# NVlabs/STEP

Measured on NVIDIA H100. Metric: clips/sec (T=32,224x224) STEP max_iter=3, higher is better.
Workload: dtype f16

## Files before the change

step_b200/build.py:

```python
import os
import subprocess
import sys
from concurrent.futures import ThreadPoolExecutor

HERE = os.path.dirname(os.path.abspath(__file__))
CSRC = os.path.join(HERE, "csrc")
OBJ = os.path.join(HERE, "_obj")
LIB = os.path.join(HERE, "libstep_b200.so")
NVCC = os.environ.get("NVCC", "/usr/local/cuda/bin/nvcc")
SOURCES = ["api.cu", "nms.cu", "roi.cu", "tubes.cu", "pool_layout.cu", "conv_simt.cu", "conv_umma.cu", "conv_halo.cu", "bottleneck_exit.cu", "train.cu", "optim.cu"]
FLAGS = ["-gencode", "arch=compute_90a,code=sm_90a", "-O3", "-std=c++17", "-lineinfo",
         "-Xcompiler", "-fPIC", "-Xptxas", "-v"]
NO_FMAD = {"nms.cu", "roi.cu", "tubes.cu", "train.cu", "optim.cu"}


def _deps(src):
    return [os.path.join(CSRC, src), os.path.join(CSRC, "common.cuh"), os.path.join(CSRC, "umma_ptx.cuh"),
            os.path.join(os.path.dirname(HERE), "include", "step_b200.h")]


def _stale(target, deps):
    if not os.path.exists(target):
        return True
    t = os.path.getmtime(target)
    return any(os.path.getmtime(d) > t for d in deps)


def _compile(src, verbose):
    obj = os.path.join(OBJ, src.replace(".cu", ".o"))
    if not _stale(obj, _deps(src)):
        return obj, ""
    cmd = [NVCC] + FLAGS + (["-fmad=false"] if src in NO_FMAD else []) + ["-c", os.path.join(CSRC, src), "-o", obj]
    r = subprocess.run(cmd, capture_output=True, text=True)
    if r.returncode != 0:
        raise RuntimeError("nvcc failed for %s:\n%s\n%s" % (src, r.stdout, r.stderr))
    return obj, r.stderr


def build(verbose=False):
    os.makedirs(OBJ, exist_ok=True)
    with ThreadPoolExecutor(max_workers=min(8, len(SOURCES))) as ex:
        res = list(ex.map(lambda s: _compile(s, verbose), SOURCES))
    objs = [o for o, _ in res]
    if verbose:
        for _, log in res:
            if log:
                print(log)
    if _stale(LIB, objs):
        cmd = [NVCC, "-shared"] + FLAGS[:2] + ["-o", LIB] + objs + ["-lcudart"]
        r = subprocess.run(cmd, capture_output=True, text=True)
        if r.returncode != 0:
            raise RuntimeError("link failed:\n%s\n%s" % (r.stdout, r.stderr))
    return LIB


if __name__ == "__main__":
    print(build(verbose="-v" in sys.argv))
```

step_b200/csrc/api.cu:

```cuda
#include <stdarg.h>
#include <string.h>

#include <atomic>

#include <stdlib.h>

#include "common.cuh"

namespace step {

static thread_local char g_err[512] = "";
static std::atomic<uint64_t> g_launches{0};

char* err_buf() { return g_err; }
void count_launch() { g_launches.fetch_add(1, std::memory_order_relaxed); }

int fail(int code, const char* fmt, ...) {
  va_list ap;
  va_start(ap, fmt);
  vsnprintf(g_err, sizeof(g_err), fmt, ap);
  va_end(ap);
  return code ? code : STEP_E_ARG;
}

int conv3d_simt_launch(const step_conv_params* p, step_stream_t stream);
int conv3d_umma_launch(const step_conv_params* p, step_stream_t stream);
int conv3d_halo_launch(const step_conv_params* p, step_stream_t stream);
bool conv3d_halo_supported(const step_conv_params* p);

}

using namespace step;

extern "C" int step_version(void) { return 100; }
extern "C" const char* step_last_error(void) { return g_err; }
extern "C" uint64_t step_launch_count(void) { return g_launches.load(std::memory_order_relaxed); }

extern "C" int step_conv3d_fwd(const step_conv_params* p, step_stream_t stream) {
  STEP_CHECK_ARG(p != nullptr, "conv3d: null params");
  STEP_CHECK_ARG(p->dtype == STEP_F32 || p->dtype == STEP_F16, "conv3d: bad dtype %d", p->dtype);
  STEP_CHECK_ARG(p->x && p->w && p->y, "conv3d: null tensor pointer");
  STEP_CHECK_ARG(p->N > 0 && p->T > 0 && p->H > 0 && p->W > 0 && p->Cin > 0 && p->Cout > 0, "conv3d: bad extent");
  STEP_CHECK_ARG(p->KT > 0 && p->KH > 0 && p->KW > 0 && p->ST > 0 && p->SH > 0 && p->SW > 0, "conv3d: bad filter/stride");
  STEP_CHECK_ARG(p->OT > 0 && p->OH > 0 && p->OW > 0, "conv3d: bad output extent");
  STEP_CHECK_ARG(p->n_splits >= 0 && p->n_splits <= 2, "conv3d: bad n_splits");
  STEP_CHECK_ARG(p->n_splits > 0 || p->out_ld >= p->out_coff + p->Cout, "conv3d: output slice [%d,%d) exceeds out_ld %d",
                 p->out_coff, p->out_coff + p->Cout, p->out_ld);
  STEP_CHECK_ARG(p->n_splits == 0 || (p->dtype == STEP_F16 && p->a_mode != 9), "conv3d: fused outputs are f16 tensor-core only");
  STEP_CHECK_ARG((p->OT - 1) * p->ST - p->PT < p->T && (p->OH - 1) * p->SH - p->PH < p->H && (p->OW - 1) * p->SW - p->PW < p->W,
                 "conv3d: output extent inconsistent with input/stride/pad");
  if (p->dtype == STEP_F32 || p->a_mode == 9) return conv3d_simt_launch(p, stream);
  if (p->a_mode == 4) {
    STEP_CHECK_ARG(p->ST == 1 && p->SH == 1 && p->SW == 1 && conv3d_halo_supported(p), "conv3d: a_mode 4 (halo) does not fit this problem");
    return conv3d_halo_launch(p, stream);
  }
  if (p->a_mode == 5) {
    static const bool halo_on = !(getenv("STEP_B200_HALO") && getenv("STEP_B200_HALO")[0] == '0');
    const int taps = p->KT * p->KH * p->KW;
    const int small = p->OH < p->OW ? p->OH : p->OW;
    if (halo_on && taps > 1 && p->ST == 1 && p->SH == 1 && p->SW == 1 && conv3d_halo_supported(p) &&
        p->Cin <= 32 && small >= 14)
      return conv3d_halo_launch(p, stream);
    step_conv_params q = *p;
    q.a_mode = taps == 1 ? 0 : 3;
    return conv3d_umma_launch(&q, stream);
  }
  return conv3d_umma_launch(p, stream);
}
```

step_b200/csrc/umma_ptx.cuh:

```cuda
#pragma once
#include <cuda.h>
#include <cuda_fp16.h>
#include <stdint.h>

namespace step {

__device__ __forceinline__ uint32_t smem_u32(const void* p) { return (uint32_t)__cvta_generic_to_shared(p); }

__device__ __forceinline__ void mbar_init(uint64_t* bar, uint32_t count) {
  asm volatile("mbarrier.init.shared::cta.b64 [%0], %1;" ::"r"(smem_u32(bar)), "r"(count));
}
__device__ __forceinline__ void mbar_expect_tx(uint64_t* bar, uint32_t bytes) {
  asm volatile("mbarrier.arrive.expect_tx.shared::cta.b64 _, [%0], %1;" ::"r"(smem_u32(bar)), "r"(bytes) : "memory");
}
__device__ __forceinline__ void mbar_arrive(uint64_t* bar) {
  asm volatile("mbarrier.arrive.shared::cta.b64 _, [%0];" ::"r"(smem_u32(bar)) : "memory");
}
__device__ __forceinline__ void mbar_wait(uint64_t* bar, uint32_t parity) {
  asm volatile(
      "{\n\t.reg .pred p;\n\t"
      "WAIT_LOOP:\n\t"
      "mbarrier.try_wait.parity.shared::cta.b64 p, [%0], %1;\n\t"
      "@p bra.uni WAIT_DONE;\n\t"
      "bra.uni WAIT_LOOP;\n\t"
      "WAIT_DONE:\n\t}" ::"r"(smem_u32(bar)), "r"(parity) : "memory");
}
__device__ __forceinline__ void fence_barrier_init() { asm volatile("fence.mbarrier_init.release.cluster;" ::: "memory"); }
__device__ __forceinline__ void fence_proxy_async() { asm volatile("fence.proxy.async.shared::cta;" ::: "memory"); }
__device__ __forceinline__ void named_sync(int id, int n) { asm volatile("bar.sync %0, %1;" ::"r"(id), "r"(n) : "memory"); }

__device__ __forceinline__ void tma_load_2d(const CUtensorMap* map, uint64_t* bar, void* dst, int c0, int c1) {
  asm volatile("cp.async.bulk.tensor.2d.shared::cluster.global.mbarrier::complete_tx::bytes [%0], [%1, {%3, %4}], [%2];"
               ::"r"(smem_u32(dst)), "l"(map), "r"(smem_u32(bar)), "r"(c0), "r"(c1) : "memory");
}
__device__ __forceinline__ void tma_load_3d(const CUtensorMap* map, uint64_t* bar, void* dst, int c0, int c1, int c2) {
  asm volatile("cp.async.bulk.tensor.3d.shared::cluster.global.mbarrier::complete_tx::bytes [%0], [%1, {%3, %4, %5}], [%2];"
               ::"r"(smem_u32(dst)), "l"(map), "r"(smem_u32(bar)), "r"(c0), "r"(c1), "r"(c2) : "memory");
}
__device__ __forceinline__ void tma_load_5d(const CUtensorMap* map, uint64_t* bar, void* dst, int c0, int c1, int c2,
                                            int c3, int c4) {
  asm volatile("cp.async.bulk.tensor.5d.shared::cluster.global.mbarrier::complete_tx::bytes [%0], [%1, {%3, %4, %5, %6, %7}], [%2];"
               ::"r"(smem_u32(dst)), "l"(map), "r"(smem_u32(bar)), "r"(c0), "r"(c1), "r"(c2), "r"(c3), "r"(c4) : "memory");
}
__device__ __forceinline__ void tma_load_im2col_5d(const CUtensorMap* map, uint64_t* bar, void* dst, int c, int w, int h,
                                                   int d, int n, uint16_t ow, uint16_t oh, uint16_t od) {
  asm volatile("cp.async.bulk.tensor.5d.shared::cluster.global.im2col.mbarrier::complete_tx::bytes [%0], [%1, {%3, %4, %5, %6, %7}], [%2], {%8, %9, %10};"
               ::"r"(smem_u32(dst)), "l"(map), "r"(smem_u32(bar)), "r"(c), "r"(w), "r"(h), "r"(d), "r"(n), "h"(ow), "h"(oh), "h"(od) : "memory");
}
__device__ __forceinline__ void tma_store_2d(const CUtensorMap* map, const void* src, int c0, int c1) {
  asm volatile("cp.async.bulk.tensor.2d.global.shared::cta.bulk_group [%0, {%2, %3}], [%1];"
               ::"l"(map), "r"(smem_u32(src)), "r"(c0), "r"(c1) : "memory");
}
__device__ __forceinline__ void bulk_commit() { asm volatile("cp.async.bulk.commit_group;" ::: "memory"); }
template <int N>
__device__ __forceinline__ void bulk_wait_read() { asm volatile("cp.async.bulk.wait_group.read %0;" ::"n"(N) : "memory"); }

template <int BK>
__device__ __forceinline__ uint64_t desc_hi_kmajor() {
  constexpr uint64_t sw = BK == 64 ? 1 : (BK == 32 ? 2 : 3);
  return (1ULL << 16) | ((uint64_t)((8 * BK * 2) >> 4) << 32) | (sw << 62);
}
__device__ __forceinline__ uint64_t desc_lo(const void* p) { return (uint64_t)((smem_u32(p) & 0x3FFFF) >> 4); }

__device__ __forceinline__ void wg_fence() { asm volatile("wgmma.fence.sync.aligned;" ::: "memory"); }
__device__ __forceinline__ void wg_commit() { asm volatile("wgmma.commit_group.sync.aligned;" ::: "memory"); }
template <int N>
__device__ __forceinline__ void wg_wait() { asm volatile("wgmma.wait_group.sync.aligned %0;" ::"n"(N) : "memory"); }

template <int N>
__device__ __forceinline__ void wgmma_f16(float* d, uint64_t da, uint64_t db, uint32_t accumulate);

#define STEP_D4(i) "+f"(d[4 * (i)]), "+f"(d[4 * (i) + 1]), "+f"(d[4 * (i) + 2]), "+f"(d[4 * (i) + 3])
#define STEP_WGMMA_F16(N, IA, IB, IC, REGS, ...)                                                                        \
  template <>                                                                                                          \
  __device__ __forceinline__ void wgmma_f16<N>(float* d, uint64_t da, uint64_t db, uint32_t accumulate) {              \
    asm volatile("{\n\t.reg .pred p;\n\tsetp.ne.b32 p, %" #IC ", 0;\n\t"                                              \
                 "wgmma.mma_async.sync.aligned.m64n" #N "k16.f32.f16.f16 {" REGS "}, %" #IA ", %" #IB ", p, 1, 1, 0, 0;\n\t}" \
                 : __VA_ARGS__ : "l"(da), "l"(db), "r"(accumulate));                                                    \
  }
STEP_WGMMA_F16(32, 16, 17, 18,
               "%0, %1, %2, %3, %4, %5, %6, %7, %8, %9, %10, %11, %12, %13, %14, %15",
               STEP_D4(0), STEP_D4(1), STEP_D4(2), STEP_D4(3))
STEP_WGMMA_F16(64, 32, 33, 34,
               "%0, %1, %2, %3, %4, %5, %6, %7, %8, %9, %10, %11, %12, %13, %14, %15, %16, %17, %18, %19, %20, %21, %22, "
               "%23, %24, %25, %26, %27, %28, %29, %30, %31",
               STEP_D4(0), STEP_D4(1), STEP_D4(2), STEP_D4(3), STEP_D4(4), STEP_D4(5), STEP_D4(6), STEP_D4(7))
STEP_WGMMA_F16(128, 64, 65, 66,
               "%0, %1, %2, %3, %4, %5, %6, %7, %8, %9, %10, %11, %12, %13, %14, %15, %16, %17, %18, %19, %20, %21, %22, "
               "%23, %24, %25, %26, %27, %28, %29, %30, %31, %32, %33, %34, %35, %36, %37, %38, %39, %40, %41, %42, %43, "
               "%44, %45, %46, %47, %48, %49, %50, %51, %52, %53, %54, %55, %56, %57, %58, %59, %60, %61, %62, %63",
               STEP_D4(0), STEP_D4(1), STEP_D4(2), STEP_D4(3), STEP_D4(4), STEP_D4(5), STEP_D4(6), STEP_D4(7),
               STEP_D4(8), STEP_D4(9), STEP_D4(10), STEP_D4(11), STEP_D4(12), STEP_D4(13), STEP_D4(14), STEP_D4(15))
STEP_WGMMA_F16(144, 72, 73, 74,
               "%0, %1, %2, %3, %4, %5, %6, %7, %8, %9, %10, %11, %12, %13, %14, %15, %16, %17, %18, %19, %20, %21, %22, "
               "%23, %24, %25, %26, %27, %28, %29, %30, %31, %32, %33, %34, %35, %36, %37, %38, %39, %40, %41, %42, %43, "
               "%44, %45, %46, %47, %48, %49, %50, %51, %52, %53, %54, %55, %56, %57, %58, %59, %60, %61, %62, %63, %64, "
               "%65, %66, %67, %68, %69, %70, %71",
               STEP_D4(0), STEP_D4(1), STEP_D4(2), STEP_D4(3), STEP_D4(4), STEP_D4(5), STEP_D4(6), STEP_D4(7),
               STEP_D4(8), STEP_D4(9), STEP_D4(10), STEP_D4(11), STEP_D4(12), STEP_D4(13), STEP_D4(14), STEP_D4(15),
               STEP_D4(16), STEP_D4(17))
STEP_WGMMA_F16(152, 76, 77, 78,
               "%0, %1, %2, %3, %4, %5, %6, %7, %8, %9, %10, %11, %12, %13, %14, %15, %16, %17, %18, %19, %20, %21, %22, "
               "%23, %24, %25, %26, %27, %28, %29, %30, %31, %32, %33, %34, %35, %36, %37, %38, %39, %40, %41, %42, %43, "
               "%44, %45, %46, %47, %48, %49, %50, %51, %52, %53, %54, %55, %56, %57, %58, %59, %60, %61, %62, %63, %64, "
               "%65, %66, %67, %68, %69, %70, %71, %72, %73, %74, %75",
               STEP_D4(0), STEP_D4(1), STEP_D4(2), STEP_D4(3), STEP_D4(4), STEP_D4(5), STEP_D4(6), STEP_D4(7),
               STEP_D4(8), STEP_D4(9), STEP_D4(10), STEP_D4(11), STEP_D4(12), STEP_D4(13), STEP_D4(14), STEP_D4(15),
               STEP_D4(16), STEP_D4(17), STEP_D4(18))
STEP_WGMMA_F16(160, 80, 81, 82,
               "%0, %1, %2, %3, %4, %5, %6, %7, %8, %9, %10, %11, %12, %13, %14, %15, %16, %17, %18, %19, %20, %21, %22, "
               "%23, %24, %25, %26, %27, %28, %29, %30, %31, %32, %33, %34, %35, %36, %37, %38, %39, %40, %41, %42, %43, "
               "%44, %45, %46, %47, %48, %49, %50, %51, %52, %53, %54, %55, %56, %57, %58, %59, %60, %61, %62, %63, %64, "
               "%65, %66, %67, %68, %69, %70, %71, %72, %73, %74, %75, %76, %77, %78, %79",
               STEP_D4(0), STEP_D4(1), STEP_D4(2), STEP_D4(3), STEP_D4(4), STEP_D4(5), STEP_D4(6), STEP_D4(7),
               STEP_D4(8), STEP_D4(9), STEP_D4(10), STEP_D4(11), STEP_D4(12), STEP_D4(13), STEP_D4(14), STEP_D4(15),
               STEP_D4(16), STEP_D4(17), STEP_D4(18), STEP_D4(19))
STEP_WGMMA_F16(176, 88, 89, 90,
               "%0, %1, %2, %3, %4, %5, %6, %7, %8, %9, %10, %11, %12, %13, %14, %15, %16, %17, %18, %19, %20, %21, %22, "
               "%23, %24, %25, %26, %27, %28, %29, %30, %31, %32, %33, %34, %35, %36, %37, %38, %39, %40, %41, %42, %43, "
               "%44, %45, %46, %47, %48, %49, %50, %51, %52, %53, %54, %55, %56, %57, %58, %59, %60, %61, %62, %63, %64, "
               "%65, %66, %67, %68, %69, %70, %71, %72, %73, %74, %75, %76, %77, %78, %79, %80, %81, %82, %83, %84, %85, "
               "%86, %87",
               STEP_D4(0), STEP_D4(1), STEP_D4(2), STEP_D4(3), STEP_D4(4), STEP_D4(5), STEP_D4(6), STEP_D4(7),
               STEP_D4(8), STEP_D4(9), STEP_D4(10), STEP_D4(11), STEP_D4(12), STEP_D4(13), STEP_D4(14), STEP_D4(15),
               STEP_D4(16), STEP_D4(17), STEP_D4(18), STEP_D4(19), STEP_D4(20), STEP_D4(21))
STEP_WGMMA_F16(192, 96, 97, 98,
               "%0, %1, %2, %3, %4, %5, %6, %7, %8, %9, %10, %11, %12, %13, %14, %15, %16, %17, %18, %19, %20, %21, %22, "
               "%23, %24, %25, %26, %27, %28, %29, %30, %31, %32, %33, %34, %35, %36, %37, %38, %39, %40, %41, %42, %43, "
               "%44, %45, %46, %47, %48, %49, %50, %51, %52, %53, %54, %55, %56, %57, %58, %59, %60, %61, %62, %63, %64, "
               "%65, %66, %67, %68, %69, %70, %71, %72, %73, %74, %75, %76, %77, %78, %79, %80, %81, %82, %83, %84, %85, "
               "%86, %87, %88, %89, %90, %91, %92, %93, %94, %95",
               STEP_D4(0), STEP_D4(1), STEP_D4(2), STEP_D4(3), STEP_D4(4), STEP_D4(5), STEP_D4(6), STEP_D4(7),
               STEP_D4(8), STEP_D4(9), STEP_D4(10), STEP_D4(11), STEP_D4(12), STEP_D4(13), STEP_D4(14), STEP_D4(15),
               STEP_D4(16), STEP_D4(17), STEP_D4(18), STEP_D4(19), STEP_D4(20), STEP_D4(21), STEP_D4(22), STEP_D4(23))
STEP_WGMMA_F16(208, 104, 105, 106,
               "%0, %1, %2, %3, %4, %5, %6, %7, %8, %9, %10, %11, %12, %13, %14, %15, %16, %17, %18, %19, %20, %21, %22, "
               "%23, %24, %25, %26, %27, %28, %29, %30, %31, %32, %33, %34, %35, %36, %37, %38, %39, %40, %41, %42, %43, "
               "%44, %45, %46, %47, %48, %49, %50, %51, %52, %53, %54, %55, %56, %57, %58, %59, %60, %61, %62, %63, %64, "
               "%65, %66, %67, %68, %69, %70, %71, %72, %73, %74, %75, %76, %77, %78, %79, %80, %81, %82, %83, %84, %85, "
               "%86, %87, %88, %89, %90, %91, %92, %93, %94, %95, %96, %97, %98, %99, %100, %101, %102, %103",
               STEP_D4(0), STEP_D4(1), STEP_D4(2), STEP_D4(3), STEP_D4(4), STEP_D4(5), STEP_D4(6), STEP_D4(7),
               STEP_D4(8), STEP_D4(9), STEP_D4(10), STEP_D4(11), STEP_D4(12), STEP_D4(13), STEP_D4(14), STEP_D4(15),
               STEP_D4(16), STEP_D4(17), STEP_D4(18), STEP_D4(19), STEP_D4(20), STEP_D4(21), STEP_D4(22), STEP_D4(23),
               STEP_D4(24), STEP_D4(25))
STEP_WGMMA_F16(224, 112, 113, 114,
               "%0, %1, %2, %3, %4, %5, %6, %7, %8, %9, %10, %11, %12, %13, %14, %15, %16, %17, %18, %19, %20, %21, %22, "
               "%23, %24, %25, %26, %27, %28, %29, %30, %31, %32, %33, %34, %35, %36, %37, %38, %39, %40, %41, %42, %43, "
               "%44, %45, %46, %47, %48, %49, %50, %51, %52, %53, %54, %55, %56, %57, %58, %59, %60, %61, %62, %63, %64, "
               "%65, %66, %67, %68, %69, %70, %71, %72, %73, %74, %75, %76, %77, %78, %79, %80, %81, %82, %83, %84, %85, "
               "%86, %87, %88, %89, %90, %91, %92, %93, %94, %95, %96, %97, %98, %99, %100, %101, %102, %103, %104, "
               "%105, %106, %107, %108, %109, %110, %111",
               STEP_D4(0), STEP_D4(1), STEP_D4(2), STEP_D4(3), STEP_D4(4), STEP_D4(5), STEP_D4(6), STEP_D4(7),
               STEP_D4(8), STEP_D4(9), STEP_D4(10), STEP_D4(11), STEP_D4(12), STEP_D4(13), STEP_D4(14), STEP_D4(15),
               STEP_D4(16), STEP_D4(17), STEP_D4(18), STEP_D4(19), STEP_D4(20), STEP_D4(21), STEP_D4(22), STEP_D4(23),
               STEP_D4(24), STEP_D4(25), STEP_D4(26), STEP_D4(27))
STEP_WGMMA_F16(256, 128, 129, 130,
               "%0, %1, %2, %3, %4, %5, %6, %7, %8, %9, %10, %11, %12, %13, %14, %15, %16, %17, %18, %19, %20, %21, %22, "
               "%23, %24, %25, %26, %27, %28, %29, %30, %31, %32, %33, %34, %35, %36, %37, %38, %39, %40, %41, %42, %43, "
               "%44, %45, %46, %47, %48, %49, %50, %51, %52, %53, %54, %55, %56, %57, %58, %59, %60, %61, %62, %63, %64, "
               "%65, %66, %67, %68, %69, %70, %71, %72, %73, %74, %75, %76, %77, %78, %79, %80, %81, %82, %83, %84, %85, "
               "%86, %87, %88, %89, %90, %91, %92, %93, %94, %95, %96, %97, %98, %99, %100, %101, %102, %103, %104, "
               "%105, %106, %107, %108, %109, %110, %111, %112, %113, %114, %115, %116, %117, %118, %119, %120, %121, "
               "%122, %123, %124, %125, %126, %127",
               STEP_D4(0), STEP_D4(1), STEP_D4(2), STEP_D4(3), STEP_D4(4), STEP_D4(5), STEP_D4(6), STEP_D4(7),
               STEP_D4(8), STEP_D4(9), STEP_D4(10), STEP_D4(11), STEP_D4(12), STEP_D4(13), STEP_D4(14), STEP_D4(15),
               STEP_D4(16), STEP_D4(17), STEP_D4(18), STEP_D4(19), STEP_D4(20), STEP_D4(21), STEP_D4(22), STEP_D4(23),
               STEP_D4(24), STEP_D4(25), STEP_D4(26), STEP_D4(27), STEP_D4(28), STEP_D4(29), STEP_D4(30), STEP_D4(31))
#undef STEP_WGMMA_F16

template <int N>
__device__ __forceinline__ void wgmma_f16_ra(float* d, const uint32_t* a, uint64_t db, uint32_t accumulate);
template <>
__device__ __forceinline__ void wgmma_f16_ra<256>(float* d, const uint32_t* a, uint64_t db, uint32_t accumulate) {
  asm volatile("{\n\t.reg .pred p;\n\tsetp.ne.b32 p, %133, 0;\n\t"
               "wgmma.mma_async.sync.aligned.m64n256k16.f32.f16.f16 {"
               "%0, %1, %2, %3, %4, %5, %6, %7, %8, %9, %10, %11, %12, %13, %14, %15, %16, %17, %18, %19, %20, %21, %22, "
               "%23, %24, %25, %26, %27, %28, %29, %30, %31, %32, %33, %34, %35, %36, %37, %38, %39, %40, %41, %42, %43, "
               "%44, %45, %46, %47, %48, %49, %50, %51, %52, %53, %54, %55, %56, %57, %58, %59, %60, %61, %62, %63, %64, "
               "%65, %66, %67, %68, %69, %70, %71, %72, %73, %74, %75, %76, %77, %78, %79, %80, %81, %82, %83, %84, %85, "
               "%86, %87, %88, %89, %90, %91, %92, %93, %94, %95, %96, %97, %98, %99, %100, %101, %102, %103, %104, "
               "%105, %106, %107, %108, %109, %110, %111, %112, %113, %114, %115, %116, %117, %118, %119, %120, %121, "
               "%122, %123, %124, %125, %126, %127}, {%128, %129, %130, %131}, %132, p, 1, 1, 0;\n\t}"
               : STEP_D4(0), STEP_D4(1), STEP_D4(2), STEP_D4(3), STEP_D4(4), STEP_D4(5), STEP_D4(6), STEP_D4(7),
                 STEP_D4(8), STEP_D4(9), STEP_D4(10), STEP_D4(11), STEP_D4(12), STEP_D4(13), STEP_D4(14), STEP_D4(15),
                 STEP_D4(16), STEP_D4(17), STEP_D4(18), STEP_D4(19), STEP_D4(20), STEP_D4(21), STEP_D4(22), STEP_D4(23),
                 STEP_D4(24), STEP_D4(25), STEP_D4(26), STEP_D4(27), STEP_D4(28), STEP_D4(29), STEP_D4(30), STEP_D4(31)
               : "r"(a[0]), "r"(a[1]), "r"(a[2]), "r"(a[3]), "l"(db), "r"(accumulate));
}
#undef STEP_D4

__device__ __forceinline__ void wgmma_64x64(float* d, uint64_t da, uint64_t db, uint32_t accumulate) {
  wgmma_f16<64>(d, da, db, accumulate);
}

template <int R>
__device__ __forceinline__ void setmaxnreg_dec() { asm volatile("setmaxnreg.dec.sync.aligned.u32 %0;" ::"n"(R)); }
template <int R>
__device__ __forceinline__ void setmaxnreg_inc() { asm volatile("setmaxnreg.inc.sync.aligned.u32 %0;" ::"n"(R)); }

__device__ __forceinline__ void pdl_wait() { asm volatile("griddepcontrol.wait;" ::: "memory"); }
__device__ __forceinline__ void pdl_launch_dependents() { asm volatile("griddepcontrol.launch_dependents;" ::: "memory"); }

__device__ __forceinline__ bool elect_one() {
  uint32_t pred;
  asm volatile(
      "{\n\t.reg .pred p;\n\t"
      "elect.sync _|p, 0xffffffff;\n\t"
      "selp.u32 %0, 1, 0, p;\n\t}"
      : "=r"(pred));
  return pred != 0;
}


}
```

step_b200/i3d.py:

```python
import torch

from . import _lib as L
from . import engine as E
from .engine import Act


def get_padding_shape(filter_shape, stride):
    pads = [E.same_pad(k, s) for k, s in zip(filter_shape, stride)]
    return pads[1] + pads[2] + pads[0]


class Unit3Dpy(torch.nn.Module):

    def __init__(self, in_channels, out_channels, kernel_size=(1, 1, 1), stride=(1, 1, 1), activation='relu',
                 padding='SAME', use_bias=False, use_bn=True):
        super(Unit3Dpy, self).__init__()
        if padding not in ('SAME', 'VALID'):
            raise ValueError('padding should be in [VALID|SAME] but got {}'.format(padding))
        self.padding = padding
        self.activation = activation
        self.use_bn = use_bn
        self.kernel_size = tuple(kernel_size)
        self.stride = tuple(stride)
        self.conv3d = torch.nn.Conv3d(in_channels, out_channels, kernel_size, stride=stride, bias=use_bias)
        if use_bn:
            self.batch3d = torch.nn.BatchNorm3d(out_channels)
        self._cache = {}

    def packed(self, code, s2d=False):
        bn = self.batch3d if self.use_bn else None
        tens = [self.conv3d.weight, self.conv3d.bias] + ([bn.weight, bn.bias, bn.running_mean, bn.running_var] if bn else [])
        key = (code, s2d) + E.params_key(*tens)
        hit = self._cache.get("k")
        if hit != key:
            w = E.pack_stem_s2d(self.conv3d.weight) if s2d else E.pack_conv_weight(self.conv3d.weight, code)
            scale, shift = E.fold_bn(bn, self.conv3d.bias, self.conv3d.out_channels, w.device)
            self._cache = {"k": key, "v": (w, scale, shift)}
        return self._cache["v"]

    def out_channels(self):
        return self.conv3d.out_channels

    def forward(self, x, out=None, residual=None):
        if not isinstance(x, Act):
            raise RuntimeError("step_b200.Unit3Dpy runs on engine.Act handles; use BaseNet / TwoBranchNet")
        relu = self.activation is not None
        if self.padding == 'VALID':
            pad_lo = (0, 0, 0)
            dims = tuple((d - k) // s + 1 for d, k, s in zip((x.T, x.H, x.W), self.kernel_size, self.stride))
        else:
            pad_lo, dims = None, None
        w, scale, shift = self.packed(x.code)
        if out is None:
            od = dims or E.same_out_dims((x.T, x.H, x.W), self.kernel_size, self.stride)
            out = Act.empty(x.N, od[0], od[1], od[2], self.conv3d.out_channels, x.code, x.device)
        return E.conv(x, w, scale, shift, out, self.kernel_size, self.stride, pad_lo, relu, residual, out_dims=dims, tag=self)

    def forward_s2d(self, x_s2d):
        w, scale, shift = self.packed(L.F16, s2d=True)
        out = Act.empty(x_s2d.N, x_s2d.T, x_s2d.H, x_s2d.W, self.conv3d.out_channels, L.F16, x_s2d.device)
        return E.conv(x_s2d, w, scale, shift, out, (4, 4, 4), (1, 1, 1), (1, 1, 1), self.activation is not None,
                      a_mode=L.A_HALO if E.STEM_HALO else None, out_dims=(x_s2d.T, x_s2d.H, x_s2d.W),
                      zero_cin_last_kt=4 * self.conv3d.in_channels, tag=("s2d", self))


class MaxPool3dTFPadding(torch.nn.Module):

    def __init__(self, kernel_size, stride=None, padding='SAME'):
        super(MaxPool3dTFPadding, self).__init__()
        self.kernel_size = tuple(kernel_size)
        self.stride = tuple(stride if stride is not None else kernel_size)
        if padding == 'SAME':
            self.padding_shape = get_padding_shape(self.kernel_size, self.stride)

    def forward(self, x, out=None):
        return E.maxpool(x, self.kernel_size, self.stride, out)


class Mixed(torch.nn.Module):

    def __init__(self, in_channels, out_channels):
        super(Mixed, self).__init__()
        o = out_channels
        self.branch_0 = Unit3Dpy(in_channels, o[0], kernel_size=(1, 1, 1))
        self.branch_1 = torch.nn.Sequential(Unit3Dpy(in_channels, o[1], kernel_size=(1, 1, 1)),
                                            Unit3Dpy(o[1], o[2], kernel_size=(3, 3, 3)))
        self.branch_2 = torch.nn.Sequential(Unit3Dpy(in_channels, o[3], kernel_size=(1, 1, 1)),
                                            Unit3Dpy(o[3], o[4], kernel_size=(3, 3, 3)))
        self.branch_3 = torch.nn.Sequential(MaxPool3dTFPadding(kernel_size=(3, 3, 3), stride=(1, 1, 1), padding='SAME'),
                                            Unit3Dpy(in_channels, o[5], kernel_size=(1, 1, 1)))
        self.out_plan = (o[0], o[2], o[4], o[5])

    def out_channels(self):
        return sum(self.out_plan)

    def forward(self, x, out=None):
        c0, c1, c2, c3 = self.out_plan
        if out is None:
            out = Act.empty(x.N, x.T, x.H, x.W, c0 + c1 + c2 + c3, x.code, x.device)
        if x.code == L.F16 and E.FUSE_1X1:
            return self._forward_fused(x, out)
        E.run_parallel(
            x.device,
            lambda: self.branch_1[1](self.branch_1[0](x), out=out.slice(c0, c1)),
            [lambda: self.branch_0(x, out=out.slice(0, c0)),
             lambda: self.branch_2[1](self.branch_2[0](x), out=out.slice(c0 + c1, c2)),
             lambda: self.branch_3[1](self.branch_3[0](x), out=out.slice(c0 + c1 + c2, c3))])
        return out


    def _fused_weights(self):
        units = (self.branch_0, self.branch_1[0], self.branch_2[0])
        parts = [u.packed(L.F16) for u in units]
        key = tuple(id(p[0]) for p in parts)
        c = self.__dict__.get("_fused")
        if c is None or c[0] != key:
            w = torch.cat([p[0] for p in parts], 0).contiguous()
            scale = torch.cat([p[1] for p in parts]).contiguous()
            shift = torch.cat([p[2] for p in parts]).contiguous()
            self.__dict__["_fused"] = (key, (w, scale, shift))
            c = self.__dict__["_fused"]
        return c[1]

    def _forward_fused(self, x, out):
        c0, c1, c2, c3 = self.out_plan
        w, scale, shift = self._fused_weights()
        m1 = self.branch_1[0].conv3d.out_channels
        m2 = self.branch_2[0].conv3d.out_channels
        t1 = Act.empty(x.N, x.T, x.H, x.W, m1, x.code, x.device)
        t2 = Act.empty(x.N, x.T, x.H, x.W, m2, x.code, x.device)

        def trunk():
            E.conv(x, w, scale, shift, out.slice(0, c0), (1, 1, 1), extra_outs=[t1, t2],
                   tag=[self.branch_0, self.branch_1[0], self.branch_2[0]])

        def tail():
            E.run_parallel(x.device,
                           lambda: self.branch_1[1](t1, out=out.slice(c0, c1)),
                           [lambda: self.branch_2[1](t2, out=out.slice(c0 + c1, c2))])
        E.run_parallel(x.device, lambda: (trunk(), tail()),
                       [lambda: self.branch_3[1](self.branch_3[0](x), out=out.slice(c0 + c1 + c2, c3))],
                       first_side=2)
        return out


class I3D_head(torch.nn.Module):

    def __init__(self):
        super(I3D_head, self).__init__()
        self.maxPool3d = MaxPool3dTFPadding(kernel_size=(1, 3, 3), stride=(1, 2, 2), padding='SAME')
        self.mixed_5b = Mixed(832, [256, 160, 320, 32, 128, 128])
        self.mixed_5c = Mixed(832, [384, 192, 384, 48, 128, 128])


def build_trunk_stages():
    return [
        Unit3Dpy(out_channels=64, in_channels=3, kernel_size=(7, 7, 7), stride=(2, 2, 2), padding='SAME'),
        MaxPool3dTFPadding(kernel_size=(1, 3, 3), stride=(1, 2, 2), padding='SAME'),
        Unit3Dpy(out_channels=64, in_channels=64, kernel_size=(1, 1, 1), padding='SAME'),
        Unit3Dpy(out_channels=192, in_channels=64, kernel_size=(3, 3, 3), padding='SAME'),
        MaxPool3dTFPadding(kernel_size=(1, 3, 3), stride=(1, 2, 2), padding='SAME'),
        Mixed(192, [64, 96, 128, 16, 32, 32]),
        Mixed(256, [128, 128, 192, 32, 96, 64]),
        MaxPool3dTFPadding(kernel_size=(3, 3, 3), stride=(2, 2, 2), padding='SAME'),
        Mixed(480, [192, 96, 208, 16, 48, 64]),
        Mixed(512, [160, 112, 224, 24, 64, 64]),
        Mixed(512, [128, 128, 256, 24, 64, 64]),
        Mixed(512, [112, 144, 288, 32, 64, 64]),
        Mixed(528, [256, 160, 320, 32, 128, 128]),
    ]
```

Before: 1089.

## Add dedicated warp-specialized WGMMA kernel for space-to-depth stem convolution

Adds a specialized stem conv kernel for the 7x7x7 stem after space-to-depth (Cin=24, 4x4x4 taps, 64 outputs). A TMA producer warp loads the input halo patch and streams the weights through a 6-stage mbarrier ring. Two consumer warpgroups run WGMMA directly on the shifted patch descriptors and write the epilogue through stmatrix staging. The Python side slices the s2d input to the real 24 channels, so the zero-padded last-kt channels are skipped. The halo path now dispatches to this kernel when the shape matches, adding a highly shape-specific code path.

Measured after the change: 1132, median of 6. +3.9%, better.

```diff
diff --git a/step_b200/build.py b/step_b200/build.py
--- a/step_b200/build.py
+++ b/step_b200/build.py
@@ -8,7 +8,7 @@
 OBJ = os.path.join(HERE, "_obj")
 LIB = os.path.join(HERE, "libstep_b200.so")
 NVCC = os.environ.get("NVCC", "/usr/local/cuda/bin/nvcc")
-SOURCES = ["api.cu", "nms.cu", "roi.cu", "tubes.cu", "pool_layout.cu", "conv_simt.cu", "conv_umma.cu", "conv_halo.cu", "bottleneck_exit.cu", "train.cu", "optim.cu"]
+SOURCES = ["api.cu", "nms.cu", "roi.cu", "tubes.cu", "pool_layout.cu", "conv_simt.cu", "conv_umma.cu", "conv_halo.cu", "conv_stem.cu", "bottleneck_exit.cu", "train.cu", "optim.cu"]
 FLAGS = ["-gencode", "arch=compute_90a,code=sm_90a", "-O3", "-std=c++17", "-lineinfo",
          "-Xcompiler", "-fPIC", "-Xptxas", "-v"]
 NO_FMAD = {"nms.cu", "roi.cu", "tubes.cu", "train.cu", "optim.cu"}
diff --git a/step_b200/csrc/api.cu b/step_b200/csrc/api.cu
--- a/step_b200/csrc/api.cu
+++ b/step_b200/csrc/api.cu
@@ -27,6 +27,8 @@
 int conv3d_umma_launch(const step_conv_params* p, step_stream_t stream);
 int conv3d_halo_launch(const step_conv_params* p, step_stream_t stream);
 bool conv3d_halo_supported(const step_conv_params* p);
+int conv3d_stem_launch(const step_conv_params* p, step_stream_t stream);
+bool conv3d_stem_supported(const step_conv_params* p);
 
 }
 
@@ -51,6 +53,7 @@
                  "conv3d: output extent inconsistent with input/stride/pad");
   if (p->dtype == STEP_F32 || p->a_mode == 9) return conv3d_simt_launch(p, stream);
   if (p->a_mode == 4) {
+    if (conv3d_stem_supported(p)) return conv3d_stem_launch(p, stream);
     STEP_CHECK_ARG(p->ST == 1 && p->SH == 1 && p->SW == 1 && conv3d_halo_supported(p), "conv3d: a_mode 4 (halo) does not fit this problem");
     return conv3d_halo_launch(p, stream);
   }
diff --git a/step_b200/csrc/conv_stem.cu b/step_b200/csrc/conv_stem.cu
--- /dev/null
+++ b/step_b200/csrc/conv_stem.cu
@@ -0,0 +1,230 @@
+#include <cuda.h>
+#include <stdlib.h>
+#include <string.h>
+
+#include "common.cuh"
+#include "umma_ptx.cuh"
+
+namespace step {
+
+constexpr int kStemThreads = 384;
+constexpr int kStemTT = 4, kStemTH = 16, kStemTW = 8;
+constexpr int kStemGroups = 3;
+constexpr int kStemHpT = kStemTT + 3, kStemHpH = kStemTH + 3, kStemHpW = kStemTW + 3;
+constexpr int kStemPlanePix = kStemHpH * kStemHpW;
+constexpr int kStemChunk = (kStemHpT * kStemPlanePix * 16 + 127) / 128 * 128;
+constexpr int kStemBlock = 64 * 16;
+constexpr int kStemStageBytes = kStemGroups * 8 * kStemBlock;
+constexpr int kStemStages = 6;
+constexpr int kStemSteps = 8;
+constexpr int kStemBook = 1024;
+constexpr int kStemPitch = 144;
+constexpr int kStemSmem = kStemBook + 1024 + kStemStages * kStemStageBytes + kStemGroups * kStemChunk;
+static_assert(kStemSmem <= 227 * 1024, "stem kernel exceeds shared memory");
+static_assert(kStemTT * kStemTH * kStemTW * kStemPitch <= kStemStages * kStemStageBytes, "staging tile exceeds the ring");
+constexpr uint64_t kStemAHi = ((uint64_t)((4 * kStemBlock) >> 4) << 16) | ((uint64_t)(128 >> 4) << 32);
+constexpr uint64_t kStemBHi = ((uint64_t)((kStemHpW * 16) >> 4) << 16) | ((uint64_t)((kStemHpW * 16) >> 4) << 32);
+
+struct StemGeom {
+  int OT, OH, OW, tiles_w, tiles_h, tiles_t;
+  int out_ld, out_coff, relu;
+};
+
+template <int NG>
+__device__ __forceinline__ void stem_mma_stage(float (&acc)[2][64], uint64_t a_lo, uint64_t b_lo) {
+#pragma unroll
+  for (int kw = 0; kw < 4; ++kw)
+#pragma unroll
+    for (int gi = 0; gi < NG; ++gi)
+#pragma unroll
+      for (int j = 0; j < 2; ++j)
+        wgmma_f16<128>(acc[j], kStemAHi | (a_lo + (uint64_t)((gi * 8 + kw) * (kStemBlock >> 4))),
+                       kStemBHi | (b_lo + (uint64_t)(gi * (kStemChunk >> 4) + j * kStemPlanePix + kw)), 1u);
+}
+
+template <int NG>
+__device__ __forceinline__ void stem_stage(float (&acc)[2][64], int st, int wg, bool leader, uint8_t* ring, uint8_t* patch,
+                                           uint64_t* full_bar, uint64_t* empty_bar) {
+  const int s = st % kStemStages;
+  mbar_wait(&full_bar[s], (uint32_t)(st / kStemStages) & 1u);
+  const int kt = st >> 1, kh0 = (st & 1) * 2;
+  const uint64_t a_lo = desc_lo(ring + (size_t)s * kStemStageBytes);
+  const uint64_t b_lo = desc_lo(patch) + (uint64_t)((2 * wg + kt) * kStemPlanePix + kh0 * kStemHpW);
+  wg_fence();
+  stem_mma_stage<NG>(acc, a_lo, b_lo);
+  wg_commit();
+  wg_wait<1>();
+  if (st > 0 && leader) mbar_arrive(&empty_bar[(st - 1) % kStemStages]);
+}
+
+__global__ void __launch_bounds__(kStemThreads, 1)
+conv_stem_kernel(const __grid_constant__ CUtensorMap map_x, const __grid_constant__ CUtensorMap map_w, StemGeom g,
+                 const float* __restrict__ scale, const float* __restrict__ shift, __half* __restrict__ y) {
+  extern __shared__ __align__(1024) uint8_t smem_raw[];
+  uint64_t* full_bar = (uint64_t*)smem_raw;
+  uint64_t* empty_bar = full_bar + kStemStages;
+  uint64_t* pfull_bar = empty_bar + kStemStages;
+  uint8_t* ring = (uint8_t*)(((uintptr_t)smem_raw + kStemBook + 1023) & ~(uintptr_t)1023);
+  uint8_t* patch = ring + kStemStages * kStemStageBytes;
+
+  const int warp = threadIdx.x >> 5, lane = threadIdx.x & 31;
+  int b = blockIdx.x;
+  const int tw = b % g.tiles_w; b /= g.tiles_w;
+  const int th = b % g.tiles_h; b /= g.tiles_h;
+  const int tt = b % g.tiles_t;
+  const int n = b / g.tiles_t;
+
+  if (threadIdx.x == 0) {
+    asm volatile("prefetch.tensormap [%0];" ::"l"(&map_x) : "memory");
+    asm volatile("prefetch.tensormap [%0];" ::"l"(&map_w) : "memory");
+    for (int s = 0; s < kStemStages; ++s) { mbar_init(&full_bar[s], 1); mbar_init(&empty_bar[s], 2); }
+    mbar_init(pfull_bar, 1);
+    fence_barrier_init();
+  }
+  __syncthreads();
+  pdl_wait();
+  pdl_launch_dependents();
+
+  if (warp < 4) {
+    setmaxnreg_dec<40>();
+    if (warp == 0 && elect_one()) {
+      mbar_expect_tx(pfull_bar, (uint32_t)(kStemGroups * kStemHpT * kStemPlanePix * 16));
+      for (int c = 0; c < kStemGroups; ++c)
+        tma_load_5d(&map_x, pfull_bar, patch + (size_t)c * kStemChunk, c * 8, tw * kStemTW - 1, th * kStemTH - 1,
+                    tt * kStemTT - 1, n);
+      for (int st = 0; st < kStemSteps; ++st) {
+        const int s = st % kStemStages, use = st / kStemStages;
+        if (use > 0) mbar_wait(&empty_bar[s], (uint32_t)(use - 1) & 1u);
+        const int ng = st < kStemSteps - 2 ? kStemGroups : kStemGroups - 1;
+        mbar_expect_tx(&full_bar[s], (uint32_t)(ng * 8 * kStemBlock));
+        uint8_t* dst = ring + (size_t)s * kStemStageBytes;
+        for (int c = 0; c < ng; ++c)
+          for (int j = 0; j < 8; ++j)
+            tma_load_3d(&map_w, &full_bar[s], dst + (c * 8 + j) * kStemBlock, c * 8, st * 8 + j, 0);
+      }
+    }
+  } else {
+    setmaxnreg_inc<232>();
+    const int wg = (warp >> 2) - 1;
+    const int ct = threadIdx.x - 128;
+    const bool leader = ct % 128 == 0;
+    float acc[2][64];
+#pragma unroll
+    for (int j = 0; j < 2; ++j)
+#pragma unroll
+      for (int i = 0; i < 64; ++i) acc[j][i] = 0.0f;
+    mbar_wait(pfull_bar, 0);
+    for (int st = 0; st < kStemSteps - 2; ++st) stem_stage<kStemGroups>(acc, st, wg, leader, ring, patch, full_bar, empty_bar);
+    for (int st = kStemSteps - 2; st < kStemSteps; ++st)
+      stem_stage<kStemGroups - 1>(acc, st, wg, leader, ring, patch, full_bar, empty_bar);
+    wg_wait<0>();
+    const int co = (warp & 3) * 16 + (lane >> 2);
+    float sc[2], sh[2];
+#pragma unroll
+    for (int i = 0; i < 2; ++i) {
+      sc[i] = scale ? scale[co + 8 * i] : 1.0f;
+      sh[i] = shift ? shift[co + 8 * i] : 0.0f;
+    }
+    named_sync(1, 256);
+    const int m = lane >> 3;
+    const uint32_t lane_addr = smem_u32(ring) + (uint32_t)(((m >> 1) * 8 + (lane & 7)) * kStemPitch +
+                                                           ((warp & 3) * 16 + (m & 1) * 8) * 2);
+#pragma unroll
+    for (int j = 0; j < 2; ++j)
+#pragma unroll
+      for (int q = 0; q < 16; q += 2) {
+        uint32_t v[4];
+#pragma unroll
+        for (int mm = 0; mm < 4; ++mm) {
+          const int qq = q + (mm >> 1), i = mm & 1;
+          float f0 = fmaf(acc[j][4 * qq + 2 * i], sc[i], sh[i]);
+          float f1 = fmaf(acc[j][4 * qq + 2 * i + 1], sc[i], sh[i]);
+          if (g.relu) { f0 = fmaxf(f0, 0.0f); f1 = fmaxf(f1, 0.0f); }
+          const __half2 h2 = __floats2half2_rn(f0, f1);
+          v[mm] = *reinterpret_cast<const uint32_t*>(&h2);
+        }
+        stmatrix_x4_trans(lane_addr + (uint32_t)(((2 * wg + j) * 128 + q * 8) * kStemPitch), v);
+      }
+    named_sync(1, 256);
+#pragma unroll 4
+    for (int i = ct; i < kStemTT * kStemTH * kStemTW * 8; i += 256) {
+      const int pix = i >> 3, ch = i & 7;
+      const int ot = tt * kStemTT + (pix >> 7), oh = th * kStemTH + ((pix >> 3) & 15), ow = tw * kStemTW + (pix & 7);
+      if (ot >= g.OT || oh >= g.OH || ow >= g.OW) continue;
+      const uint4 val = *reinterpret_cast<const uint4*>(ring + (size_t)pix * kStemPitch + ch * 16);
+      *reinterpret_cast<uint4*>(y + ((((size_t)n * g.OT + ot) * g.OH + oh) * g.OW + ow) * g.out_ld + g.out_coff + ch * 8) = val;
+    }
+  }
+}
+
+typedef CUresult (*StemEncodeTiledFn)(CUtensorMap*, CUtensorMapDataType, cuuint32_t, void*, const cuuint64_t*, const cuuint64_t*,
+                                      const cuuint32_t*, const cuuint32_t*, CUtensorMapInterleave, CUtensorMapSwizzle,
+                                      CUtensorMapL2promotion, CUtensorMapFloatOOBfill);
+static StemEncodeTiledFn g_stem_encode = nullptr;
+
+bool conv3d_stem_supported(const step_conv_params* p) {
+  return p->dtype == STEP_F16 && p->Cin == 24 && p->Cout == 64 && p->KT == 4 && p->KH == 4 && p->KW == 4 && p->ST == 1 &&
+         p->SH == 1 && p->SW == 1 && p->PT == 1 && p->PH == 1 && p->PW == 1 && p->OT == p->T && p->OH == p->H &&
+         p->OW == p->W && !p->residual && p->n_splits == 0 && p->zero_cin_last_kt > 0 && p->zero_cin_last_kt <= 16;
+}
+
+int conv3d_stem_launch(const step_conv_params* p, step_stream_t stream) {
+  STEP_CHECK_ARG(conv3d_stem_supported(p), "conv3d(stem): unsupported problem");
+  STEP_CHECK_ARG((((uintptr_t)p->x | (uintptr_t)p->w | (uintptr_t)p->y) & 15) == 0 && p->in_ld % 8 == 0 && p->in_ld >= 24 &&
+                 p->w_ld % 8 == 0 && p->w_ld >= 24 && p->out_ld % 8 == 0 && p->out_coff % 8 == 0, "conv3d(stem): alignment");
+  if (!g_stem_encode) {
+    cudaDriverEntryPointQueryResult q;
+    void* f = nullptr;
+    if (cudaGetDriverEntryPoint("cuTensorMapEncodeTiled", &f, cudaEnableDefault, &q) != cudaSuccess || !f)
+      return fail(STEP_E_DRIVER, "cuTensorMapEncodeTiled entry point unavailable");
+    g_stem_encode = (StemEncodeTiledFn)f;
+  }
+  StemGeom g;
+  memset(&g, 0, sizeof(g));
+  g.OT = p->OT; g.OH = p->OH; g.OW = p->OW;
+  g.out_ld = p->out_ld; g.out_coff = p->out_coff; g.relu = p->relu;
+  g.tiles_w = (p->OW + kStemTW - 1) / kStemTW; g.tiles_h = (p->OH + kStemTH - 1) / kStemTH;
+  g.tiles_t = (p->OT + kStemTT - 1) / kStemTT;
+  const long long ctas = (long long)p->N * g.tiles_t * g.tiles_h * g.tiles_w;
+  STEP_CHECK_ARG(ctas < (1LL << 31), "conv3d(stem): grid too large");
+  const cuuint32_t ones[5] = {1, 1, 1, 1, 1};
+  CUtensorMap mx, mw;
+  {
+    cuuint64_t dims[5] = {24, (cuuint64_t)p->W, (cuuint64_t)p->H, (cuuint64_t)p->T, (cuuint64_t)p->N};
+    cuuint64_t strides[4] = {(cuuint64_t)p->in_ld * 2, (cuuint64_t)p->W * p->in_ld * 2, (cuuint64_t)p->H * p->W * p->in_ld * 2,
+                             (cuuint64_t)p->T * p->H * p->W * p->in_ld * 2};
+    cuuint32_t box[5] = {8, (cuuint32_t)kStemHpW, (cuuint32_t)kStemHpH, (cuuint32_t)kStemHpT, 1};
+    CUresult cr = g_stem_encode(&mx, CU_TENSOR_MAP_DATA_TYPE_FLOAT16, 5, (void*)p->x, dims, strides, box, ones,
+                                CU_TENSOR_MAP_INTERLEAVE_NONE, CU_TENSOR_MAP_SWIZZLE_NONE, CU_TENSOR_MAP_L2_PROMOTION_L2_128B,
+                                CU_TENSOR_MAP_FLOAT_OOB_FILL_NONE);
+    if (cr != CUDA_SUCCESS) return fail(STEP_E_DRIVER, "conv3d(stem): tensor map (patch) encode failed: CUresult %d", (int)cr);
+  }
+  {
+    cuuint64_t dims[3] = {24, 64, 64};
+    cuuint64_t strides[2] = {(cuuint64_t)p->w_ld * 2, (cuuint64_t)64 * p->w_ld * 2};
+    cuuint32_t box[3] = {8, 1, 64};
+    CUresult cr = g_stem_encode(&mw, CU_TENSOR_MAP_DATA_TYPE_FLOAT16, 3, (void*)p->w, dims, strides, box, ones,
+                                CU_TENSOR_MAP_INTERLEAVE_NONE, CU_TENSOR_MAP_SWIZZLE_NONE, CU_TENSOR_MAP_L2_PROMOTION_L2_256B,
+                                CU_TENSOR_MAP_FLOAT_OOB_FILL_NONE);
+    if (cr != CUDA_SUCCESS) return fail(STEP_E_DRIVER, "conv3d(stem): tensor map (weights) encode failed: CUresult %d", (int)cr);
+  }
+  static std::atomic<unsigned long long> attr_seen{0};
+  if (first_use_on_device(attr_seen)) {
+    cudaError_t e = cudaFuncSetAttribute(conv_stem_kernel, cudaFuncAttributeMaxDynamicSharedMemorySize, kStemSmem);
+    if (e != cudaSuccess) return fail((int)e, "conv_stem_kernel attribute: %s", cudaGetErrorString(e));
+  }
+  cudaLaunchConfig_t cfg = {};
+  cudaLaunchAttribute attr[1];
+  cfg.gridDim = dim3((unsigned)ctas); cfg.blockDim = dim3(kStemThreads); cfg.dynamicSmemBytes = kStemSmem; cfg.stream = cu(stream);
+  if (pdl_enabled()) {
+    attr[0].id = cudaLaunchAttributeProgrammaticStreamSerialization;
+    attr[0].val.programmaticStreamSerializationAllowed = 1;
+    cfg.attrs = attr; cfg.numAttrs = 1;
+  }
+  cudaError_t le = cudaLaunchKernelEx(&cfg, conv_stem_kernel, mx, mw, g, p->scale, p->shift, (__half*)p->y);
+  if (le != cudaSuccess) { cudaGetLastError(); return fail((int)le, "conv_stem_kernel launch: %s", cudaGetErrorString(le)); }
+  STEP_LAUNCH_CHECK("conv_stem_kernel");
+  return 0;
+}
+
+}
diff --git a/step_b200/csrc/umma_ptx.cuh b/step_b200/csrc/umma_ptx.cuh
--- a/step_b200/csrc/umma_ptx.cuh
+++ b/step_b200/csrc/umma_ptx.cuh
@@ -50,6 +50,10 @@
 __device__ __forceinline__ void tma_store_2d(const CUtensorMap* map, const void* src, int c0, int c1) {
   asm volatile("cp.async.bulk.tensor.2d.global.shared::cta.bulk_group [%0, {%2, %3}], [%1];"
                ::"l"(map), "r"(smem_u32(src)), "r"(c0), "r"(c1) : "memory");
+}
+__device__ __forceinline__ void stmatrix_x4_trans(uint32_t addr, const uint32_t* v) {
+  asm volatile("stmatrix.sync.aligned.m8n8.x4.trans.shared.b16 [%0], {%1, %2, %3, %4};"
+               ::"r"(addr), "r"(v[0]), "r"(v[1]), "r"(v[2]), "r"(v[3]) : "memory");
 }
 __device__ __forceinline__ void bulk_commit() { asm volatile("cp.async.bulk.commit_group;" ::: "memory"); }
 template <int N>
diff --git a/step_b200/i3d.py b/step_b200/i3d.py
--- a/step_b200/i3d.py
+++ b/step_b200/i3d.py
@@ -59,7 +59,8 @@
     def forward_s2d(self, x_s2d):
         w, scale, shift = self.packed(L.F16, s2d=True)
         out = Act.empty(x_s2d.N, x_s2d.T, x_s2d.H, x_s2d.W, self.conv3d.out_channels, L.F16, x_s2d.device)
-        return E.conv(x_s2d, w, scale, shift, out, (4, 4, 4), (1, 1, 1), (1, 1, 1), self.activation is not None,
+        x = x_s2d.slice(0, 8 * self.conv3d.in_channels)
+        return E.conv(x, w, scale, shift, out, (4, 4, 4), (1, 1, 1), (1, 1, 1), self.activation is not None,
                       a_mode=L.A_HALO if E.STEM_HALO else None, out_dims=(x_s2d.T, x_s2d.H, x_s2d.W),
                       zero_cin_last_kt=4 * self.conv3d.in_channels, tag=("s2d", self))
 
```
